# simon3dv/SLR-SFS

Measured on AMD Instinct MI355X. Metric: synthesised frames/sec at 768x1280 N=60, higher is better.
Workload: dtype f32 (convs: fp32 in/out/accumulate, operands 2 x f16 splits = 22 bits; all-fp32: fps_fp32_convs); 1 GPU; C3 baseline pipeline, 768x1280, N=60, random weights; parallelism=1 GPU, no collective, collective_bytes_received_per_rank_per_clip=0

## Files before the change

include/slr_splat.h:

```cpp
#ifndef SLR_SPLAT_H
#define SLR_SPLAT_H

#include <stddef.h>

#ifdef __cplusplus
extern "C" {
#endif

#define SLR_ABI_VERSION 28

#define SLR_E_BADARG   (-1)
#define SLR_E_WORKSPACE (-2)

#define SLR_MODE_SUMMATION 0
#define SLR_MODE_AVERAGE   1
#define SLR_MODE_LINEAR    2
#define SLR_MODE_SOFTMAX   3

#define SLR_NORM_ZERO_TO_ONE 0
#define SLR_NORM_CLAMP_EPS   1

int         slr_abi_version(void);
const char *slr_last_error(void);

void slr_splat_time_next(void *ev_start, void *ev_stop);


int slr_euler_integrate(const float *motion, int H, int W, int nsteps, float sign,
                        float *disp, float *visible, void *stream);

int slr_euler_integrate_all(const float *motion, int H, int W, int nmax, float sign,
                            float *disp_all, float *vis_all, void *stream);
// ... 114 lines not shown
                      int N, int C, int H, int W,
                      void *ws, size_t ws_bytes, int prebinned, void *stream);


int slr_bn_relu_mask(const float *x, const float *scale, const float *shift, const float *mask,
                     int mask_channels, float *y, int N, int C, int H, int W, void *stream);

int slr_pconv_epilogue(const float *raw0, const float *bias, const float *mask_box, float mask_scale,
                       const float *residual, const float *next_scale, const float *next_shift,
                       float *out, float *um_out, float winsize, int N, int C, int H, int W, void *stream);

int slr_conv_saturation_count(unsigned long long *count, int reset, void *stream);
int slr_conv_saturation_record(unsigned *host_slot, void *stream);


#define SLR_CONV_IN_B8  1
#define SLR_CONV_OUT_B8 2
#define SLR_CONV_RES_B8 4
#define SLR_CONV_F32    8
#define SLR_CONV_WINO   16
#define SLR_CONV_SKIP_B8 32
#define SLR_CONV_POOL_OUT 64
#define SLR_CONV_UP_OUT 128

size_t slr_conv3x3_weight_bytes(int Cout, int Cin);
int slr_conv3x3_split_weights(const float *w , void *wsplit, int Cout, int Cin,
                              float wscale, void *stream);
int slr_conv3x3_f32_weights(const float *w , void *wfrag , int Cout, int Cin,
                            void *stream);
size_t slr_conv3x3_wino_weight_bytes(int Cout, int Cin);
int slr_conv3x3_wino_weights(const float *w , void *wfrag , int Cout, int Cin,
                             void *stream);

int slr_conv3x3_forward(const float *in, const void *wsplit, const float *bias, const float *residual, float *out,
                        int N, int Cin, int Cout, int H, int W, float wscale, float xscale,
                        const float *pre_scale, const float *pre_shift, int layout, void *stream);

int slr_pconv3x3_forward(const float *x, const float *pre_scale, const float *pre_shift, const float *mask,
                         const void *wsplit, float wscale, float xscale, const float *bias, const float *residual,
                         const float *next_scale, const float *next_shift, float *out, float *um_out,
                         int N, int Cin, int Cout, int H, int W, int layout, void *stream);

size_t slr_conv_pool_ws_bytes(int N, int Cout, int H, int W);
size_t slr_conv_up_ws_bytes(int N, int Cout, int H, int W);
int slr_conv3x3_forward_skip(const float *in, const void *wsplit, const float *bias, float *out,
                             int N, int Cin, int Cout, int H, int W, float wscale, float xscale,
// ... 280 lines not shown
```

slr-sfs_amd/_lib.py:

```python
import ctypes
import os
import threading

import torch

_HERE = os.path.dirname(os.path.abspath(__file__))
LIB_PATH = os.environ.get("SLR_SFS_AMD_LIB") or os.path.join(_HERE, "lib", "libslrsplat.so")
ABI_VERSION = 28
WS_PREBINNED, WS_CLEAN = 1, 2
BLEND_DETERMINISTIC = 1

_vp, _fp, _i, _f, _sz = ctypes.c_void_p, ctypes.c_void_p, ctypes.c_int, ctypes.c_float, ctypes.c_size_t
SIGNATURES = {
    "slr_abi_version": (_i, []),
    "slr_last_error": (ctypes.c_char_p, []),
    "slr_splat_time_next": (None, [_vp, _vp]),
    "slr_euler_integrate": (_i, [_fp, _i, _i, _i, _f, _fp, _fp, _vp]),
    "slr_euler_integrate_all": (_i, [_fp, _i, _i, _i, _f, _fp, _fp, _vp]),
    "slr_euler_backward": (_i, [_fp, _i, _i, _i, _f, _fp, _fp, _vp]),
    "slr_euler_integrate_batch": (_i, [_fp, _vp, _i, _i, _i, _f, _fp, _fp, _vp]),
    "slr_euler_backward_batch": (_i, [_fp, _vp, _i, _i, _i, _f, _fp, _fp, _vp]),
    "slr_euler_pair_forward": (_i, [_fp, _vp, _vp, _i, _i, _i, _fp, _fp, _fp, _fp, _vp]),
    "slr_euler_pair_workspace_bytes": (_sz, [_i, _i, _i]),
    "slr_euler_pair_backward": (_i, [_fp, _vp, _vp, _i, _i, _i, _fp, _fp, _fp, _vp, _sz, _vp]),
    "slr_splat_workspace_bytes": (_sz, [_i, _i, _i]),
    "slr_splat_workspace_init": (_i, [_vp, _sz, _i, _i, _i, _vp]),
    "slr_splat_bin": (_i, [_fp, _i, _i, _i, _vp, _sz, _vp]),
    "slr_splat_bin_pair": (_i, [_fp, _fp, _i, _i, _i, _vp, _vp, _sz, _vp]),
    "slr_splat_set_scan_max_tiles": (_i, [_i]),
    "slr_splat_set_front_end": (_i, [_i]),
    "slr_splat_set_scan_shape": (None, [_i, _i, _i, _i]),
# ... 3 lines not shown
    "slr_synth_group": (_i, [_fp, _fp, _fp, _i, _fp, _fp, _f, _fp, _fp, _i, _i, _i, _f, _vp, _vp, _sz, _vp]),
    "slr_clip_plan_bytes": (_sz, [_i, _i, _i]),
    "slr_clip_plan_totals": (_i, [_i, _i, _i, ctypes.POINTER(ctypes.c_size_t), ctypes.POINTER(ctypes.c_int)]),
    "slr_clip_plan_build": (_i, [_fp, _vp, _fp, _vp, _i, _i, _i, _vp, _sz, _vp]),
    "slr_pack_planes4": (_i, [_fp, _fp, _i, _i, _i, _i, _vp]),
    "slr_synth_group_clip_batch": (_i, [_fp, _fp, _fp, _i, _vp, _vp, _vp, _vp, _vp, _i, _i, _i, _f, _vp, _sz, _i, _vp, _i, _vp, _vp]),
    "slr_synth_two_groups_clip_batch": (_i, [_fp, _fp, _fp, _i, _fp, _fp, _i, _vp, _vp, _vp, _vp, _vp, _i, _i, _i, _f, _vp, _sz, _i, _vp, _i, _vp, _vp]),
    "slr_synth_group_clip": (_i, [_fp, _fp, _fp, _i, _fp, _fp, _f, _fp, _fp, _i, _i, _i, _f, _vp, _sz, _i, _i, _i, _vp]),
    "slr_global_max": (_i, [_fp, _sz, _fp, _fp, _vp]),
    "slr_softsplat_backward": (_i, [_fp, _fp, _fp, _fp, _fp, _i, _i, _i, _i, _vp]),
    "slr_softsplat_backward_ws_bytes": (_sz, [_i, _i, _i, _i]),
    "slr_softsplat_backward_ws": (_i, [_fp, _fp, _fp, _fp, _fp, _i, _i, _i, _i, _vp, _sz, _vp]),
    "slr_splat_blend_ws_bytes": (_sz, [_i, _i, _i, _i]),
    "slr_splat_blend_forward": (_i, [_fp] * 9 + [_f, _f, _f, _fp, _fp, _i, _i, _i, _i, _vp, _sz, _i, _vp, _sz, _vp]),
    "slr_splat_blend_forward_ex": (_i, [_fp] * 9 + [_f, _f, _f, _fp, _fp, _i, _i, _i, _i, _vp, _sz, _i, _i, _vp, _sz, _vp]),
    "slr_splat_fallback_count_offset": (_sz, [_i, _i, _i]),
    "slr_splat_blend_backward": (_i, [_fp] * 9 + [_f, _f, _f] + [_fp] * 9 + [_i, _i, _i, _i, _vp, _sz, _vp]),
    "slr_maxsplat_forward": (_i, [_fp, _fp, _fp, _f, _i, _i, _i, _i, _vp, _sz, _i, _vp]),
    "slr_max_warp_norm": (_i, [_fp, _fp, _fp, _fp, _i, _i, _i, _i, _vp, _sz, _i, _vp]),
    "slr_bn_relu_mask": (_i, [_fp, _fp, _fp, _fp, _i, _fp, _i, _i, _i, _i, _vp]),
    "slr_pconv_epilogue": (_i, [_fp, _fp, _fp, _f, _fp, _fp, _fp, _fp, _fp, _f, _i, _i, _i, _i, _vp]),
    "slr_conv_saturation_count": (_i, [ctypes.POINTER(ctypes.c_ulonglong), _i, _vp]),
    "slr_conv_saturation_record": (_i, [_vp, _vp]),
    "slr_conv3x3_weight_bytes": (_sz, [_i, _i]),
    "slr_conv3x3_split_weights": (_i, [_fp, _vp, _i, _i, _f, _vp]),
    "slr_conv3x3_f32_weights": (_i, [_fp, _vp, _i, _i, _vp]),
    "slr_conv3x3_wino_weight_bytes": (_sz, [_i, _i]),
    "slr_conv3x3_wino_weights": (_i, [_fp, _vp, _i, _i, _vp]),
    "slr_conv3x3_forward": (_i, [_fp, _vp, _fp, _fp, _fp, _i, _i, _i, _i, _i, _f, _f, _fp, _fp, _i, _vp]),
    "slr_pconv3x3_forward": (_i, [_fp, _fp, _fp, _fp, _vp, _f, _f, _fp, _fp, _fp, _fp, _fp, _fp, _i, _i, _i, _i, _i, _i, _vp]),
    "slr_conv_pool_ws_bytes": (_sz, [_i, _i, _i, _i]),
    "slr_conv_up_ws_bytes": (_sz, [_i, _i, _i, _i]),
    "slr_conv3x3_forward_skip": (_i, [_fp, _vp, _fp, _fp, _i, _i, _i, _i, _i, _f, _f, _fp, _fp, _fp, _vp, _fp, _i, _f, _vp, _sz, _i, _vp]),
    "slr_pconv3x3_forward_skip": (_i, [_fp, _fp, _fp, _fp, _vp, _f, _f, _fp, _fp, _fp, _i, _i, _i, _i, _i, _fp, _vp, _i, _f, _vp, _sz, _i, _vp]),
    "slr_conv3x3_forward_skipout": (_i, [_fp, _vp, _fp, _fp, _fp, _i, _i, _i, _i, _i, _f, _f, _fp, _fp, _fp, _fp, _fp, _i, _vp]),
    "slr_pconv3x3_forward_skipout": (_i, [_fp, _fp, _fp, _fp, _vp, _f, _f, _fp, _fp, _fp, _fp, _fp, _fp, _i, _i, _i, _i, _i, _fp, _fp, _i, _vp]),
    "slr_conv_tail_weight_bytes": (_sz, [_i]),
    "slr_conv_tail_weight_source": (_i, [_i, _i, _vp, _vp, _vp, _vp]),
    "slr_conv_tail_weights": (_i, [_fp, _fp, _vp, _i, _f, _f, _vp]),
    "slr_pconv3x3_forward_tail": (_i, [_fp, _fp, _vp, _f, _f, _fp, _fp, _fp, _fp, _vp, _fp, _fp, _i, _i, _i, _i, _i, _vp]),
    "slr_narrow_gather": (_i, [_fp] * 9 + [_i, _i, _i, _i, _f, _f, _f, _vp]),
    "slr_conv1x1_weight_bytes": (_sz, [_i, _i]),
    "slr_conv1x1_split_weights": (_i, [_fp, _vp, _i, _i, _f, _vp]),
    "slr_conv1x1_f32_weights": (_i, [_fp, _vp, _i, _i, _vp]),
    "slr_conv1x1_forward": (_i, [_fp, _vp, _fp, _fp, _i, _i, _i, _i, _i, _f, _f, _i, _vp]),
    "slr_avgpool3x3s2": (_i, [_fp, _fp, _i, _i, _i, _i, _i, _vp]),
# ... 189 lines not shown
```

slr-sfs_amd/csrc/conv.hip:

```cpp
#include "slr_common.hpp"

#include <string.h>

#include <atomic>
#include <mutex>
#include <type_traits>

namespace slr {

typedef _Float16 h8 __attribute__((ext_vector_type(8)));
typedef float f16v __attribute__((ext_vector_type(16)));

constexpr int CV_W = 32, CV_H = 8;
constexpr int CV_HW = CV_W + 2, CV_HH = CV_H + 2;
constexpr int CV_NPX = CV_HW * CV_HH;
constexpr int CV_THREADS = 256;
constexpr float CV_XSCALE = 64.0f;
constexpr int CV_MAXCIN = 1024;

enum { PRE_NONE = 0, PRE_BN = 1, PRE_BN_MASK = 2, PRE_BN_NONZERO = 3 };

struct ConvArgs {
    const float *in;
    const h8 *w;
    float *out;
    int N, Cin, Cout, H, W, tiles_x, nchunk;
    float unscale;
    float xscale;
    int pre;
    const float *pre_scale, *pre_shift;
    const float *mask;
    const float *bias;
    int partial;
    float mask_scale, winsize;
    const float *residual, *next_scale, *next_shift;
    float *um_out;
    int out_b8;
    int res_b8;
// ... 2 lines not shown
    long long *trace;
#endif
    int wino_groups;
    const float *skip_in;
    const h8 *skip_w;
    const float *skip_bias;
    int skip_cin, skip_nchunk;
    float skip_unscale;
    float *pool_row, *pool_col;
    int tiles_y, resample;
    float *skip_out;
};

__host__ __device__ inline int conv_cout_tile(int Cout) { return Cout > 64 ? 128 : (Cout > 32 ? 64 : 32); }
__host__ __device__ inline int conv_cout_pad(int Cout) { const int t = conv_cout_tile(Cout); return (Cout + t - 1) / t * t; }
__host__ __device__ inline int conv_cin_pad(int Cin) { return (Cin + 15) / 16 * 16; }

}
#include "conv_few.hpp"
namespace slr {

constexpr int CV_FSTR = 352;
constexpr int CV_KSTR = 260;
template <int CPW, int WCO, bool PRE, bool INB8, bool F32 = false, bool SKIP = false, bool POOL = false, bool UPS = false, bool TAIL = false>
__global__ __launch_bounds__(CV_THREADS, 2) void conv3x3_split_kernel(ConvArgs a) {
    constexpr int WPX = 4 / WCO, PT = CV_H / WPX;
    static_assert(!TAIL || (CPW == 1 && WCO == 4 && !PRE && INB8 && !F32 && !SKIP && !POOL && !UPS), "the tail phase: one instantiation");
    static_assert(!(POOL || UPS) || (SKIP && WCO == 4 && !(POOL && UPS)), "the resampling epilogues: a wave holds all 8 rows of its channel tile");
    static_assert(!F32 || CPW == 1, "the fp32 rung runs one 32-channel tile per wave");
    static_assert(!SKIP || (CPW == 1 && INB8), "the skip phase: one tile per wave, channel-blocked main input");
    constexpr int XRAW = F32 ? 2 * 16 * CV_FSTR * 4 : 2 * 2 * 2 * CV_NPX * 16, XSKIP = !SKIP ? 0 : SLR_CONV_SKIP_FILL * (F32 ? 16 * CV_KSTR * 4 : 2 * 2 * 256 * 16);
    __shared__ __attribute__((aligned(16))) unsigned char xraw[XRAW > XSKIP ? XRAW : XSKIP];
    h8 (*xs)[2][2][CV_NPX] = reinterpret_cast<h8 (*)[2][2][CV_NPX]>(xraw);
    float (*xf)[16][CV_FSTR] = reinterpret_cast<float (*)[16][CV_FSTR]>(xraw);
    __shared__ float mpl[CV_NPX];
    __shared__ float mplB[2][CV_NPX - 256];
    __shared__ float4 pss4[2][CV_MAXCIN / 4];
    const int tid = threadIdx.x, lane = tid & 63;
    const int wave = __builtin_amdgcn_readfirstlane(tid >> 6);
    const int wc = wave % WCO, wp = wave / WCO;
    const int tx = blockIdx.x % a.tiles_x, ty = blockIdx.x / a.tiles_x;
    const int x0 = tx * CV_W, y0 = ty * CV_H;
    const int n = blockIdx.z;
    const int cot0 = (blockIdx.y * WCO + wc) * CPW;
    const int HW = a.H * a.W;
    const int nchunk = a.nchunk;
    const int cmax = a.Cin - 1;
    const float *inb = a.in + (size_t)n * a.Cin * HW;
    const int pre = a.pre;

    if (PRE) {
        float *pssw = reinterpret_cast<float *>(&pss4[0][0]);
        for (int i = tid; i < nchunk * 16; i += CV_THREADS) {
            pssw[i] = i < a.Cin ? a.pre_scale[i] * (F32 ? 1.0f : a.xscale) : 0.0f;
            pssw[CV_MAXCIN + i] = i < a.Cin ? a.pre_shift[i] * (F32 ? 1.0f : a.xscale) : 0.0f;
        }
    }

    const int gB = tid >= 84 ? 1 : 0;
    const int pB = 256 + tid - 84 * gB;
    const bool liveB = tid < 168;
    bool okA, okB;
    int offA, offB;
    {
        const int pr = tid / CV_HW, pc = tid - pr * CV_HW;
        const int gy = y0 - 1 + pr, gx = x0 - 1 + pc;
        okA = (gy >= 0) & (gy < a.H) & (gx >= 0) & (gx < a.W);
        offA = okA ? gy * a.W + gx : 0;
    }
    {
        const int pr = pB / CV_HW, pc = pB - pr * CV_HW;
        const int gy = y0 - 1 + pr, gx = x0 - 1 + pc;
        okB = liveB & (gy >= 0) & (gy < a.H) & (gx >= 0) & (gx < a.W);
        offB = okB ? gy * a.W + gx : 0;
    }
    const float unit = (PRE || F32) ? 1.0f : a.xscale;
    const float mvA = (a.mask && okA) ? a.mask[(size_t)n * HW + offA] : 0.0f;
    const float mvB = (a.mask && okB) ? a.mask[(size_t)n * HW + offB] : 0.0f;
    if (a.mask) {
        mpl[tid] = mvA;
        if (tid < CV_NPX - 256) mpl[256 + tid] = mvB;
    }
    const float mA = okA ? (pre == PRE_BN_MASK ? mvA : unit) : 0.0f;
    const float mB = okB ? (pre == PRE_BN_MASK ? mvB : unit) : 0.0f;
    float cnt[3] = {0.0f, 0.0f, 0.0f};
    const bool nonzero_mask = pre == PRE_BN_NONZERO;
    const int c8max = (a.Cin >> 3) - 1;
    auto load_round = [&](auto R, int c, float (&st)[8]) {
        if (INB8) {
            const int grp = min(c * 2 + (R.value < 2 ? R.value : gB), c8max);
            const float4 *q = reinterpret_cast<const float4 *>(inb) + ((size_t)grp * HW + (unsigned)(R.value < 2 ? offA : offB)) * 2;
            const float4 u = q[0], v = q[1];
            st[0] = u.x; st[1] = u.y; st[2] = u.z; st[3] = u.w;
            st[4] = v.x; st[5] = v.y; st[6] = v.z; st[7] = v.w;
            return;
        }
#pragma unroll
        for (int j = 0; j < 8; ++j) {
            if (R.value < 2) {
                const float *pl = inb + (size_t)min(c * 16 + R.value * 8 + j, cmax) * HW;
                st[j] = pl[(unsigned)offA];
            } else {
                st[j] = inb[(unsigned)(min(c * 16 + gB * 8 + j, cmax) * HW + offB)];
            }
        }
    };
    struct Stage { int cb; float mk0, fresh, cnt; h8 hi, lo; float f[F32 ? 8 : 1]; };
    unsigned long long sat = 0ull;
    const float *pss = reinterpret_cast<const float *>(&pss4[0][0]);
    auto stage_begin = [&](auto R, int c, Stage &g) {
        g.cb = c * 16 + (R.value < 2 ? R.value * 8 : gB * 8);
        g.mk0 = R.value < 2 ? mA : mB;
        g.cnt = 0.0f;
    };
    auto stage_value = [&](int j, Stage &g, const float (&st)[8], const float *psc = nullptr, const float *psh = nullptr) {
        const float x = st[j];
        float v;
        if (PRE) {
            const float mk = (nonzero_mask & (x == 0.0f)) ? 0.0f : g.mk0;
            v = fmaxf(x * (psc ? psc[j] : pss[g.cb + j]) - (psh ? psh[j] : pss[CV_MAXCIN + g.cb + j]), 0.0f) * mk;
            g.cnt += (g.cb + j <= cmax) ? mk : 0.0f;
        } else if (F32) {
            v = g.mk0 != 0.0f ? x : 0.0f;
        } else {
            v = x * g.mk0;
        }
        if (F32) { g.f[j] = v; return; }
        v = __builtin_amdgcn_fmed3f(v, -65472.0f, 65472.0f);
        sat |= __ballot(fabsf(v) >= 65472.0f);
        const _Float16 h = (_Float16)v;
        g.hi[j] = h;
        g.lo[j] = (_Float16)(v - (float)h);
    };
    auto stage_finish = [&](auto R, int buf, const Stage &g) {
        cnt[R.value] += g.cnt * g.fresh;
        const int dst = R.value == 0 ? tid : (R.value == 1 ? CV_NPX + tid : gB * CV_NPX + pB);
        if (F32) {
            const int ch0 = R.value < 2 ? R.value * 8 : gB * 8, px = R.value < 2 ? tid : pB;
            if (R.value < 2 || liveB) {
#pragma unroll
                for (int j = 0; j < 8; ++j) xf[buf][ch0 + j][px] = g.f[j];
            }
            return;
        }
        if (R.value < 2 || liveB) {
            (&xs[buf][0][0][0])[dst] = g.hi;
            (&xs[buf][1][0][0])[dst] = g.lo;
        }
    };
    auto store_round = [&](auto R, int buf, int c, const float (&st)[8]) {
        Stage g;
        stage_begin(R, c, g);
        g.fresh = 1.0f;
#pragma unroll
        for (int j = 0; j < 8; ++j) stage_value(j, g, st);
        stage_finish(R, buf, g);
    };
    using R0 = std::integral_constant<int, 0>;
    using R1 = std::integral_constant<int, 1>;
    using R2 = std::integral_constant<int, 2>;

    f16v acc[CPW][PT];
#pragma unroll
    for (int c = 0; c < CPW; ++c)
#pragma unroll
        for (int p = 0; p < PT; ++p)
#pragma unroll
            for (int r = 0; r < 16; ++r) acc[c][p][r] = 0.0f;

    __syncthreads();
    {
        float s0[8], s1[8], s2[8];
        load_round(R0{}, 0, s0);
        load_round(R1{}, 0, s1);
        load_round(R2{}, 0, s2);
        store_round(R0{}, 0, 0, s0);
        store_round(R1{}, 0, 0, s1);
        store_round(R2{}, 0, 0, s2);
    }
    __syncthreads();
    constexpr bool DEEP = SLR_CONV_DEEP_STAGE && WCO < 4 && !F32;
    float stx[DEEP ? 3 : 1][8];
    float (&st)[8] = stx[0];
    if (DEEP) load_round(R0{}, min(1, nchunk - 1), stx[0]);

    const int bcol = lane & 31, bgrp = lane >> 5;
    const size_t wtile = (size_t)nchunk * 9 * 2 * 64;
    const h8 *wbase = a.w + (size_t)cot0 * wtile;
    h8 a_cur[CPW][2], a_nxt[CPW][2];
    auto load_a = [&](h8 (&dst)[CPW][2], int g ) {
#pragma unroll
        for (int ct = 0; ct < CPW; ++ct) {
            const h8 *q = wbase + ct * wtile + (size_t)g * 128;
            if (F32) { dst[ct][0] = q[2u * (unsigned)lane]; dst[ct][1] = q[2u * (unsigned)lane + 1u]; continue; }
            dst[ct][0] = q[(unsigned)lane];
            dst[ct][1] = q[(unsigned)lane + 64u];
        }
    };
    load_a(a_cur, 0);
    const int glast = nchunk * 9 - 1;
    h8 a_nx2[DEEP ? CPW : 1][2];
    if (DEEP) { load_a(a_nxt, min(1, glast)); }
    constexpr int PB = PT > 4 ? 4 : PT, NB = PT / PB;
    constexpr int PSA = 2;
    for (int c = 0; c < nchunk; ++c) {
        const int buf = c & 1;
        h8 bx[2][PB];
        constexpr bool PSAHEAD = PRE && !F32;
        float psc[PSAHEAD ? 8 : 1], psh[PSAHEAD ? 8 : 1];
        const int cn = min(c + 1, nchunk - 1);
        const h8 *xh = &xs[buf][0][bgrp][0], *xl = &xs[buf][1][bgrp][0];
#pragma unroll
        for (int tap = 0; tap < 9; ++tap) {
            const int kh = tap / 3, kw = tap - kh * 3;
            asm volatile("" ::: "memory");
            if (DEEP) load_a(a_nx2, min(c * 9 + tap + 2, glast));
            else load_a(a_nxt, min(c * 9 + tap + 1, glast));
            if (DEEP) {
                if (tap == 0) load_round(R1{}, cn, stx[DEEP ? 1 : 0]);
                if (tap == 3) load_round(R2{}, cn, stx[DEEP ? 2 : 0]);
                if (tap == 6) load_round(R0{}, min(c + 2, nchunk - 1), stx[0]);
            } else {
                if (tap == 0) load_round(R0{}, cn, st);
                if (tap == 3) load_round(R1{}, cn, st);
                if (tap == 6) load_round(R2{}, cn, st);
            }
            __builtin_amdgcn_sched_barrier(0);
            const bool stage_tap = tap == 2 || tap == 5 || tap == 8;
            Stage sg;
            sg.fresh = c + 1 < nchunk ? 1.0f : 0.0f;
            if (stage_tap) {
                if (tap == 2) stage_begin(R0{}, cn, sg);
                if (tap == 5) stage_begin(R1{}, cn, sg);
                if (tap == 8) stage_begin(R2{}, cn, sg);
            }
            constexpr int NM = 3 * CPW * PT, NMB = 3 * CPW * PB;
            if constexpr (F32) {
                typedef float f8v __attribute__((ext_vector_type(8)));
                union AW { h8 h[2]; f8v f; } aw;
                aw.h[0] = a_cur[0][0]; aw.h[1] = a_cur[0][1];
                constexpr int NMF = 8 * PT;
#pragma unroll
                for (int kp = 0; kp < 8; ++kp) {
                    float bv[PT];
#pragma unroll
                    for (int k = 0; k < PT; ++k) bv[k] = xf[buf][2 * kp + bgrp][(wp * PT + k + kh) * CV_HW + kw + bcol];
#pragma unroll
                    for (int k = 0; k < PT; ++k) {
                        acc[0][k] = __builtin_amdgcn_mfma_f32_32x32x2f32(aw.f[kp], bv[k], acc[0][k], 0, 0, 0);
                        if (stage_tap) {
                            const int i = kp * PT + k;
                            const int j0 = i * 8 / NMF, j1 = (i + 1) * 8 / NMF;
                            if (j1 > j0) {
#pragma unroll
                                for (int j = j0; j < j1; ++j) stage_value(j, sg, stx[DEEP ? tap / 3 : 0]);
                                __builtin_amdgcn_sched_barrier(0);
                            }
                        }
                    }
                }
            } else {
                const int pcb = cn * 16 + (tap / 3 < 2 ? tap / 3 * 8 : gB * 8);
                auto ps_load = [&](int j) {
                    if constexpr (PSAHEAD) { psc[j] = pss[pcb + j]; psh[j] = pss[CV_MAXCIN + pcb + j]; }
                };
                auto frag = [&](int t, int b, int k) { return (wp * PT + b * PB + k + t / 3) * CV_HW + t % 3 + bcol; };
#pragma unroll
                for (int hb = 0; hb < NB; ++hb) {
                    const int q = (tap * NB + hb) & 1;
                    h8 (&bh)[PB] = bx[q], (&bl)[PB] = bx[q ^ 1];
                    if (tap == 0 && hb == 0) {
#pragma unroll
                        for (int k = 0; k < PB; ++k) {
                            bh[k] = xh[frag(0, 0, k)];
                            bl[k] = xl[frag(0, 0, k)];
                        }
                    }
                    const bool more = tap < 8 || hb + 1 < NB;
                    const int ntap = hb + 1 < NB ? tap : tap + 1, nhb = hb + 1 < NB ? hb + 1 : 0;
#pragma unroll
                    for (int ib = 0; ib < NMB; ++ib) {
                        const int part = ib / (CPW * PB), k = (ib / CPW) % PB, ct = ib % CPW;
                        const int pt = hb * PB + k, i = hb * NMB + ib;
                        const h8 av = part == 0 ? a_cur[ct][1] : a_cur[ct][0];
                        const h8 bv = part == 1 ? bl[k] : bh[k];
                        acc[ct][pt] = __builtin_amdgcn_mfma_f32_32x32x16_f16(av, bv, acc[ct][pt], 0, 0, 0);
                        if (more && ct == CPW - 1) {
                            if (part == 1) bl[k] = xh[frag(ntap, nhb, k)];
                            if (part == 2) bh[k] = xl[frag(ntap, nhb, k)];
                        }
                        if (tap % 3 == 1 && i == NM - PB - 1) {
#pragma unroll
                            for (int j = 0; j < PSA; ++j) ps_load(j);
                        }
                        if (stage_tap) {
                            const int j0 = i * 8 / NM, j1 = (i + 1) * 8 / NM;
#pragma unroll
                            for (int j = j0; j < j1; ++j) {
                                if (j + PSA < 8) ps_load(j + PSA);
                                if constexpr (PSAHEAD) stage_value(j, sg, stx[DEEP ? tap / 3 : 0], psc, psh);
                                else stage_value(j, sg, stx[DEEP ? tap / 3 : 0]);
                            }
                        }
                        __builtin_amdgcn_sched_barrier(0);
                    }
                }
            }
            if (stage_tap) {
                if (tap == 2) stage_finish(R0{}, buf ^ 1, sg);
                if (tap == 5) stage_finish(R1{}, buf ^ 1, sg);
                if (tap == 8) stage_finish(R2{}, buf ^ 1, sg);
            }
#pragma unroll
            for (int ct = 0; ct < CPW; ++ct) {
                a_cur[ct][0] = a_nxt[ct][0]; a_cur[ct][1] = a_nxt[ct][1];
                if (DEEP) { a_nxt[ct][0] = a_nx2[ct][0]; a_nxt[ct][1] = a_nx2[ct][1]; }
            }
        }
        __syncthreads();
    }

    if (pre == PRE_BN_NONZERO) {
        mpl[tid] = cnt[0] + cnt[1];
        if (liveB) mplB[gB][pB - 256] = cnt[2];
        __syncthreads();
        if (tid < CV_NPX - 256) mpl[256 + tid] = mplB[0][tid] + mplB[1][tid];
    }
    __syncthreads();

    if constexpr (SKIP) {
        constexpr int SK = SLR_CONV_SKIP_FILL;
        static_assert(SK * (F32 ? 16 * CV_KSTR * 4 : 2 * 2 * 256 * 16) <= (int)sizeof(xraw), "skip fills live in the staging buffers");
        h8 (*xk)[2][2][256] = reinterpret_cast<h8 (*)[2][2][256]>(xraw);
        float (*xkf)[16][CV_KSTR] = reinterpret_cast<float (*)[16][CV_KSTR]>(xraw);
        const int ns = a.skip_nchunk, sc8max = (a.skip_cin >> 3) - 1;
        const int spr = tid >> 5, spc = tid & 31;
        const bool sok = (y0 + spr < a.H) & (x0 + spc < a.W);
        const float smk = sok ? a.xscale : 0.0f;
        const float4 *sq = reinterpret_cast<const float4 *>(a.skip_in + (size_t)n * a.skip_cin * HW) + (size_t)(sok ? (y0 + spr) * a.W + x0 + spc : 0) * 2;
        float4 sv[SK][4];
        auto sload = [&](int s0) {
#pragma unroll
            for (int k = 0; k < SK; ++k)
#pragma unroll
                for (int g = 0; g < 2; ++g) {
                    const float4 *q = sq + (size_t)min(min(s0 + k, ns - 1) * 2 + g, sc8max) * HW * 2;
                    sv[k][2 * g] = q[0];
                    sv[k][2 * g + 1] = q[1];
                }
// ... 1131 lines not shown
    a.skip_in = sk->in; a.skip_w = (const h8 *)sk->w; a.skip_bias = sk->bias;
    a.skip_cin = sk->cin; a.skip_nchunk = conv_cin_pad(sk->cin) / 16;
    a.skip_unscale = 1.0f / (xscale * sk->wscale);
    if (pool) {
        SLR_CHECK_ARG(!(up && (layout_in & SLR_CONV_POOL_OUT)), "SLR_CONV_POOL_OUT and SLR_CONV_UP_OUT are exclusive");
        SLR_CHECK_ARG(a.out_b8 && conv_cout_tile(a.Cout) == 128, "the resampling epilogues need a channel-blocked output and more than 64 output channels");
        SLR_CHECK_ARG(!up || (long long)a.N * a.Cout * a.H * a.W < (1LL << 38), "sizes");
        SLR_CHECK_ARG(sk->pool_ws && !((uintptr_t)sk->pool_ws & 15) && sk->pool_ws_bytes >= conv_pool_ws_bytes(a.N, a.Cout, a.H, a.W, up),
                      "pool_ws: slr_conv_pool_ws_bytes / slr_conv_up_ws_bytes, 16-byte aligned");
        a.tiles_y = (a.H + CV_H - 1) / CV_H;
        a.resample = up ? 2 : 1;
        a.pool_row = (float *)sk->pool_ws;
        a.pool_col = a.pool_row + (size_t)a.N * a.Cout * a.tiles_y * a.W * (up ? 2 : 1);
    }
    return 0;
}

template <int WCO, bool PRE, bool B8, bool F32, bool SKIP, bool POOL, bool UPS>
static constexpr bool conv_split_built() {
    return !(WCO == 4 && PRE && !B8) && (B8 || !SKIP) && (!(POOL || UPS) || (SKIP && WCO == 4 && !(POOL && UPS))) &&
           !(F32 && SKIP && WCO != 4);
}

static int conv_launch(ConvArgs &a, float wscale, float xscale, int layout, hipStream_t st, bool tail = false) {
    const bool in_b8 = (layout & SLR_CONV_IN_B8) != 0, f32 = (layout & SLR_CONV_F32) != 0, wino = (layout & SLR_CONV_WINO) != 0;
    const bool pre = a.pre != PRE_NONE;
    if (int e = check_xscale(xscale)) return e;
    SLR_CHECK_ARG(!f32 || (wscale == 1.0f && xscale == 1.0f), "the fp32 rung takes no operand scales (wscale = xscale = 1)");
    SLR_CHECK_ARG(!wino || (f32 && a.Cout > CF_MAXCO), "SLR_CONV_WINO goes with SLR_CONV_F32 and more than 4 output channels");
    SLR_CHECK_ARG(!wino || !pre || a.Cin <= WN_MAXCIN, "SLR_CONV_WINO with a prologue supports Cin <= 256");
    if (wino) {
        a.tiles_x = (a.W + WN_BW - 1) / WN_BW;
        a.nchunk = conv_cin_pad(a.Cin) / 16;
        a.xscale = 1.0f; a.unscale = 1.0f;
        const int blocks = a.tiles_x * ((a.H + WN_BH - 1) / WN_BH), ngrp = wino_cout_pad(a.Cout) / 64;
        const dim3 grid((blocks + WN_SLICE - 1) / WN_SLICE * WN_SLICE * ngrp, 1, a.N);
        a.wino_groups = ngrp;
#ifdef SLR_TRACE
        a.trace = g_trace;
#endif
        if (int e = dispatch([&](auto pre_, auto b8) {
                static LdsOptIn attr;
                if (int e = lds_opt_in((const void *)conv3x3_wino_kernel<pre_, b8>, (int)WN_LDS_BYTES, attr)) return e;
                hipLaunchKernelGGL((conv3x3_wino_kernel<pre_, b8>), grid, dim3(WN_THREADS), WN_LDS_BYTES, st, a);
                return 0;
            }, pre, in_b8)) return e;
// ... 5 lines not shown
        if (int e = dispatch_int<1, 2, 3, 4>(a.Cout, [&](auto nco) {
                return dispatch([&](auto pre_, auto b8, auto skp) {
                    if constexpr (b8 || !skp) hipLaunchKernelGGL((conv3x3_few_kernel<nco, pre_, b8, skp>), grid, dim3(CF_THREADS), 0, st, a);
                    else return conv_not_built();
                    return 0;
                }, pre, in_b8, a.skip_out != nullptr);
            })) return e;
        SLR_CHECK_LAUNCH();
        return 0;
    }
    a.tiles_x = (a.W + CV_W - 1) / CV_W;
    a.nchunk = conv_cin_pad(a.Cin) / 16;
    a.xscale = xscale;
    a.unscale = 1.0f / (xscale * wscale);
    if (int e = sat_counter(&a.sat)) return e;
    if (tail) {
        hipLaunchKernelGGL((conv3x3_split_kernel<1, 4, false, true, false, false, false, false, true>),
                           dim3(a.tiles_x * ((a.H + CV_H - 1) / CV_H), 1, a.N), dim3(CV_THREADS), 0, st, a);
        SLR_CHECK_LAUNCH();
        return 0;
    }
    int ct = conv_cout_tile(a.Cout);
    if (ct == 128 && pre && !in_b8) ct = 64;
    const dim3 grid(a.tiles_x * ((a.H + CV_H - 1) / CV_H), conv_cout_pad(a.Cout) / ct, a.N);
    if (int e = dispatch_int<4, 2, 1>(ct / 32, [&](auto wco) {
            return dispatch([&](auto pre_, auto b8, auto f32_, auto skip, auto pool, auto ups) {
                if constexpr (conv_split_built<wco, pre_, b8, f32_, skip, pool, ups>())
                    hipLaunchKernelGGL((conv3x3_split_kernel<1, wco, pre_, b8, f32_, skip, pool, ups>), grid, dim3(CV_THREADS), 0, st, a);
                else return conv_not_built();
                return 0;
            }, pre, in_b8, f32, a.skip_in != nullptr, a.resample == 1, a.resample == 2);
        })) return e;
    SLR_CHECK_LAUNCH();
    if (a.resample == 2) {
        const int items = 2 * a.tiles_y * 2 * a.W + 2 * a.tiles_x * 2 * a.H;
        hipLaunchKernelGGL(upsample_fix_kernel, dim3((items + 255) / 256, a.N * (a.Cout >> 3)), dim3(256), 0, st, a.out, (const float *)a.pool_row,
                           (const float *)a.pool_col, a.Cout >> 3, a.H, a.W, a.tiles_x, a.tiles_y);
        SLR_CHECK_LAUNCH();
    } else if (a.resample == 1) {
        const int OH = (a.H - 1) / 2 + 1, OW = (a.W - 1) / 2 + 1;
        const int items = (a.tiles_y - 1) * OW + (a.tiles_x - 1) * OH;
        if (items > 0) {
            hipLaunchKernelGGL(pool_fix_kernel, dim3((items + 255) / 256, a.N * (a.Cout >> 3)), dim3(256), 0, st, a.out, (const float *)a.pool_row,
                               (const float *)a.pool_col, a.Cout >> 3, a.H, a.W, a.tiles_x, a.tiles_y);
            SLR_CHECK_LAUNCH();
        }
    }
    return 0;
}

static int conv3x3_run(bool partial, const float *x, const float *pre_scale, const float *pre_shift, const float *mask,
                       const void *wsplit, float wscale, float xscale, const float *bias, const float *residual,
                       const float *next_scale, const float *next_shift, float *out, float *um_out,
                       int N, int Cin, int Cout, int H, int W, const SkipOp *sk, int layout, void *stream) {
    SLR_CHECK_ARG(x && wsplit && (bias || !partial) && out, "null pointer");
    if (int e = conv_check_layout(layout, x, out, Cin, Cout, residual, partial && !mask)) return e;
    SLR_CHECK_ARG(!pre_scale == !pre_shift, "pre_scale / pre_shift go together");
    SLR_CHECK_ARG(!pre_scale || Cin <= CV_MAXCIN, "prologue supports Cin <= 1024");
    SLR_CHECK_ARG(!partial || mask || pre_scale, "mask = NULL (derived from x != 0) needs the raw input, i.e. pre_scale / pre_shift");
    SLR_CHECK_ARG(!next_scale == !next_shift, "next_scale / next_shift go together");
    SLR_CHECK_ARG(!(residual && next_scale), "residual and next-BN fusion are exclusive");
    if (int e = conv_check_dims(N, Cin, Cout, H, W)) return e;
    ConvArgs a = {};
    a.in = x; a.w = (const h8 *)wsplit; a.bias = bias; a.out = out;
    a.N = N; a.Cin = Cin; a.Cout = Cout; a.H = H; a.W = W;
    a.pre = !pre_scale ? PRE_NONE : !partial ? PRE_BN : mask ? PRE_BN_MASK : PRE_BN_NONZERO;
    a.pre_scale = pre_scale; a.pre_shift = pre_shift; a.mask = mask;
    if (partial) {
        a.partial = 1;
        a.mask_scale = mask ? (float)Cin : 1.0f;
        a.winsize = (float)Cin * 9.0f;
    }
    a.residual = residual; a.next_scale = next_scale; a.next_shift = next_shift; a.um_out = um_out;
    a.out_b8 = (layout & SLR_CONV_OUT_B8) != 0;
    a.res_b8 = (layout & SLR_CONV_RES_B8) != 0;
    if (int e = conv_set_skip(a, sk, xscale, layout)) return e;
    return conv_launch(a, wscale, xscale, layout, (hipStream_t)stream);
}

// ... 117 lines not shown
```

slr-sfs_amd/nets.py:

```python
import collections
import ctypes
import math
import types

import threading

import torch
import torch.nn as nn
import torch.nn.functional as F

from . import _lib


IN_B8, OUT_B8, RES_B8, CONV_F32, CONV_WINO, SKIP_B8, POOL_OUT, UP_OUT = 1, 2, 4, 8, 16, 32, 64, 128


class _Route(threading.local):
    cpu_reference = False
    torch_convs = False
    act_scale = 64.0
    f32_kernels = False
    winograd = False
    fused_skips = True
    fused_pools = True
    narrow_tail = True


_S = _Route()


def _b8(x, channels):
    return x.is_cuda and channels % 8 == 0 and not _S.torch_convs


class torch_convolutions:

    def __enter__(self):
        self._prev, _S.torch_convs = _S.torch_convs, True
        return self

    def __exit__(self, *exc):
        _S.torch_convs = self._prev
        return False


FP32_WINOGRAD = False


# ... 32 lines not shown

class staged_skips:

    def __init__(self, pools_only=False):
        self.pools_only = pools_only

    def __enter__(self):
        self._prev = (_S.fused_skips, _S.fused_pools)
        _S.fused_skips = self.pools_only
        _S.fused_pools = False

    def __exit__(self, *exc):
        _S.fused_skips, _S.fused_pools = self._prev
        return False


class staged_narrow_end:

    def __enter__(self):
        self._prev, _S.narrow_tail = _S.narrow_tail, False

    def __exit__(self, *exc):
        _S.narrow_tail = self._prev
        return False


_BlockRoute = collections.namedtuple("_BlockRoute", "form b8 first skip second pool")


def _block_route(blk, x, b8_in, explicit_mask=True):
    cout = blk.conv_aa.weight.shape[0]
    b8 = _b8(x, cout)
    lin = IN_B8 if b8_in else 0
    rides = blk.conv_b is not None and b8_in and _S.fused_skips and x.is_cuda and not _S.torch_convs
    if rides and cout <= 4 and explicit_mask:
        return _BlockRoute("narrow", b8, lin, 0, 0, False)
    first = lin | (OUT_B8 if b8 else 0)
    if rides and b8 and cout > 4 and not (_S.f32_kernels and (_S.winograd or cout <= 64)):
        return _BlockRoute("fused", b8, first, 0, IN_B8 | OUT_B8, blk.pools if (cout > 64 and _S.fused_pools) else False)
    skip_b8 = b8 and cout > 4 if blk.conv_b is not None else b8_in
    second = (IN_B8 | OUT_B8 if b8 else 0) | (RES_B8 if skip_b8 and b8 else 0)
    return _BlockRoute("staged", b8, first, lin | (OUT_B8 if skip_b8 else 0), second, False)


def _pool_out(N, cout, H, W, like, pool):
    if not pool:
# ... 102 lines not shown
        self.cin, self.k = cin, k
        nn.init.normal_(self.weight, std=math.sqrt(1.0 / (cin * k * k)))

    def forward(self, x, pre_bn=None, residual=None, layout=0):
        return self.conv(x, self.bias, pre_bn, residual, layout)

    def _w4(self):
        w = self.weight

        def make():
            w4 = torch.zeros(w.shape[1], 4, device=w.device, dtype=torch.float32)
            w4[:, :w.shape[0]] = w.view(w.shape[0], w.shape[1]).t()
            return w4.contiguous()
        return _cached(self, "_w4c", make, w)

    def _conv3x3(self, name, x, args, layout=0, pre_bn=None, next_bn=None, partial=False, skipout=False, skip_conv=None,
                 skip_b8=False, pool=False):
        N, cin, H, W = x.shape
        cout = self.weight.shape[0]
        c = types.SimpleNamespace(dims=(N, cin, cout, H, W), um=None, skip=None)
        c.buf, c.wscale, c.xscale, arith = self._split_weights()
        c.psc, c.psh = pre_bn if pre_bn is not None else (None, None)
        c.nsc, c.nsh = next_bn if next_bn is not None else (None, None)
        layout |= arith
        if skip_conv is not None:
            c.sbuf, c.swscale, _, sarith = skip_conv._split_weights()
            assert arith == sarith and not (arith & CONV_WINO)
            c.out, c.ws, c.ws_bytes, pflag = _pool_out(N, cout, H, W, x, pool)
            layout |= pflag | (SKIP_B8 if skip_b8 else 0)
        else:
            c.out = torch.empty(N, cout, H, W, device=x.device, dtype=x.dtype)
        if skipout:
            c.skip = torch.empty(N, cout, H, W, device=x.device, dtype=x.dtype)
        if partial:
            c.um = torch.empty(N, 1, H, W, device=x.device, dtype=x.dtype)
        _lib.call(name, x.device, *args(c), layout)
        return c

    def forward_skipout(self, x, pre_bn, skip_conv, layout=0):
        assert self.k == 3 and skip_conv.k == 1 and _fused_ok(x)
        c = self._conv3x3("slr_conv3x3_forward_skipout", x, lambda c: (
            x, c.buf, self.bias, None, c.out, *c.dims, c.wscale, c.xscale, c.psc, c.psh, skip_conv._w4(), skip_conv.bias, c.skip),
            layout, pre_bn, skipout=True)
        return c.out, c.skip

    def forward_skip(self, x, pre_bn, skip_x, skip_conv, layout=0, skip_b8=False, pool=False):
        assert self.k == 3 and skip_conv.k == 1 and _fused_ok(x, skip_x)
# ... 713 lines not shown
```

Before: 189.5 frames/s.

## Add 12-row tall conv tiles for 64-channel split convs on large grids

Adds a taller 32x12 spatial tile variant of the split-f16 3x3 conv kernel for 64-channel output tiles. It is chosen automatically when the grid has enough tiles per CU. The change generalises the halo staging from three to four load rounds, re-spaces the staging taps, and adjusts the MFMA pixel batching. The goal is to cut halo overhead, meaning redundant input loads and weight-fragment reloads per output pixel. The cost is more LDS and register pressure and fewer blocks, which could hurt occupancy or tail balance.

```diff
diff --git a/include/slr_splat.h b/include/slr_splat.h
--- a/include/slr_splat.h
+++ b/include/slr_splat.h
@@ -7,7 +7,7 @@
 extern "C" {
 #endif
 
-#define SLR_ABI_VERSION 28
+#define SLR_ABI_VERSION 29
 
 #define SLR_E_BADARG   (-1)
 #define SLR_E_WORKSPACE (-2)
@@ -168,6 +168,10 @@
 #define SLR_CONV_SKIP_B8 32
 #define SLR_CONV_POOL_OUT 64
 #define SLR_CONV_UP_OUT 128
+#define SLR_CONV_ROWS8 256
+#define SLR_CONV_ROWS_TALL 512
+
+int slr_conv_tile_rows(int Cout, int H, int W, int N, int layout, int num_cu);
 
 size_t slr_conv3x3_weight_bytes(int Cout, int Cin);
 int slr_conv3x3_split_weights(const float *w , void *wsplit, int Cout, int Cin,
diff --git a/slr-sfs_amd/_lib.py b/slr-sfs_amd/_lib.py
--- a/slr-sfs_amd/_lib.py
+++ b/slr-sfs_amd/_lib.py
@@ -6,7 +6,7 @@
 
 _HERE = os.path.dirname(os.path.abspath(__file__))
 LIB_PATH = os.environ.get("SLR_SFS_AMD_LIB") or os.path.join(_HERE, "lib", "libslrsplat.so")
-ABI_VERSION = 28
+ABI_VERSION = 29
 WS_PREBINNED, WS_CLEAN = 1, 2
 BLEND_DETERMINISTIC = 1
 
@@ -56,6 +56,7 @@
     "slr_pconv_epilogue": (_i, [_fp, _fp, _fp, _f, _fp, _fp, _fp, _fp, _fp, _f, _i, _i, _i, _i, _vp]),
     "slr_conv_saturation_count": (_i, [ctypes.POINTER(ctypes.c_ulonglong), _i, _vp]),
     "slr_conv_saturation_record": (_i, [_vp, _vp]),
+    "slr_conv_tile_rows": (_i, [_i] * 6),
     "slr_conv3x3_weight_bytes": (_sz, [_i, _i]),
     "slr_conv3x3_split_weights": (_i, [_fp, _vp, _i, _i, _f, _vp]),
     "slr_conv3x3_f32_weights": (_i, [_fp, _vp, _i, _i, _vp]),
diff --git a/slr-sfs_amd/csrc/conv.hip b/slr-sfs_amd/csrc/conv.hip
--- a/slr-sfs_amd/csrc/conv.hip
+++ b/slr-sfs_amd/csrc/conv.hip
@@ -12,8 +12,8 @@
 typedef float f16v __attribute__((ext_vector_type(16)));
 
 constexpr int CV_W = 32, CV_H = 8;
-constexpr int CV_HW = CV_W + 2, CV_HH = CV_H + 2;
-constexpr int CV_NPX = CV_HW * CV_HH;
+constexpr int CV_HW = CV_W + 2;
+constexpr int CV_H_TALL = 12;
 constexpr int CV_THREADS = 256;
 constexpr float CV_XSCALE = 64.0f;
 constexpr int CV_MAXCIN = 1024;
@@ -62,25 +62,32 @@
 
 constexpr int CV_FSTR = 352;
 constexpr int CV_KSTR = 260;
-template <int CPW, int WCO, bool PRE, bool INB8, bool F32 = false, bool SKIP = false, bool POOL = false, bool UPS = false, bool TAIL = false>
+template <int CPW, int WCO, bool PRE, bool INB8, bool F32 = false, bool SKIP = false, bool POOL = false, bool UPS = false, bool TAIL = false,
+          int TH = CV_H>
 __global__ __launch_bounds__(CV_THREADS, 2) void conv3x3_split_kernel(ConvArgs a) {
-    constexpr int WPX = 4 / WCO, PT = CV_H / WPX;
+    constexpr int WPX = 4 / WCO, PT = TH / WPX;
+    constexpr bool TALL = TH != CV_H;
+    constexpr int NPX = CV_HW * (TH + 2), REM = NPX - 256;
+    constexpr bool COMB = 2 * REM <= 256;
+    constexpr int NR = COMB ? 3 : 4;
+    static_assert(REM > 0 && REM <= 256, "the halo block: more than one and at most two rounds of pixels");
+    static_assert(!TALL || (CPW == 1 && WCO == 2 && !F32 && !SKIP && !POOL && !UPS && !TAIL), "the tall block: 64-channel rows of the split rung");
     static_assert(!TAIL || (CPW == 1 && WCO == 4 && !PRE && INB8 && !F32 && !SKIP && !POOL && !UPS), "the tail phase: one instantiation");
     static_assert(!(POOL || UPS) || (SKIP && WCO == 4 && !(POOL && UPS)), "the resampling epilogues: a wave holds all 8 rows of its channel tile");
     static_assert(!F32 || CPW == 1, "the fp32 rung runs one 32-channel tile per wave");
     static_assert(!SKIP || (CPW == 1 && INB8), "the skip phase: one tile per wave, channel-blocked main input");
-    constexpr int XRAW = F32 ? 2 * 16 * CV_FSTR * 4 : 2 * 2 * 2 * CV_NPX * 16, XSKIP = !SKIP ? 0 : SLR_CONV_SKIP_FILL * (F32 ? 16 * CV_KSTR * 4 : 2 * 2 * 256 * 16);
+    constexpr int XRAW = F32 ? 2 * 16 * CV_FSTR * 4 : 2 * 2 * 2 * NPX * 16, XSKIP = !SKIP ? 0 : SLR_CONV_SKIP_FILL * (F32 ? 16 * CV_KSTR * 4 : 2 * 2 * 256 * 16);
     __shared__ __attribute__((aligned(16))) unsigned char xraw[XRAW > XSKIP ? XRAW : XSKIP];
-    h8 (*xs)[2][2][CV_NPX] = reinterpret_cast<h8 (*)[2][2][CV_NPX]>(xraw);
+    h8 (*xs)[2][2][NPX] = reinterpret_cast<h8 (*)[2][2][NPX]>(xraw);
     float (*xf)[16][CV_FSTR] = reinterpret_cast<float (*)[16][CV_FSTR]>(xraw);
-    __shared__ float mpl[CV_NPX];
-    __shared__ float mplB[2][CV_NPX - 256];
+    __shared__ float mpl[NPX];
+    __shared__ float mplB[2][COMB ? REM : 1];
     __shared__ float4 pss4[2][CV_MAXCIN / 4];
     const int tid = threadIdx.x, lane = tid & 63;
     const int wave = __builtin_amdgcn_readfirstlane(tid >> 6);
     const int wc = wave % WCO, wp = wave / WCO;
     const int tx = blockIdx.x % a.tiles_x, ty = blockIdx.x / a.tiles_x;
-    const int x0 = tx * CV_W, y0 = ty * CV_H;
+    const int x0 = tx * CV_W, y0 = ty * TH;
     const int n = blockIdx.z;
     const int cot0 = (blockIdx.y * WCO + wc) * CPW;
     const int HW = a.H * a.W;
@@ -97,9 +104,9 @@
         }
     }
 
-    const int gB = tid >= 84 ? 1 : 0;
-    const int pB = 256 + tid - 84 * gB;
-    const bool liveB = tid < 168;
+    const int gB = COMB && tid >= REM ? 1 : 0;
+    const int pB = 256 + tid - REM * gB;
+    const bool liveB = tid < (COMB ? 2 * REM : REM);
     bool okA, okB;
     int offA, offB;
     {
@@ -119,16 +126,16 @@
     const float mvB = (a.mask && okB) ? a.mask[(size_t)n * HW + offB] : 0.0f;
     if (a.mask) {
         mpl[tid] = mvA;
-        if (tid < CV_NPX - 256) mpl[256 + tid] = mvB;
+        if (tid < REM) mpl[256 + tid] = mvB;
     }
     const float mA = okA ? (pre == PRE_BN_MASK ? mvA : unit) : 0.0f;
     const float mB = okB ? (pre == PRE_BN_MASK ? mvB : unit) : 0.0f;
-    float cnt[3] = {0.0f, 0.0f, 0.0f};
+    float cnt[NR] = {};
     const bool nonzero_mask = pre == PRE_BN_NONZERO;
     const int c8max = (a.Cin >> 3) - 1;
     auto load_round = [&](auto R, int c, float (&st)[8]) {
         if (INB8) {
-            const int grp = min(c * 2 + (R.value < 2 ? R.value : gB), c8max);
+            const int grp = min(c * 2 + (R.value < 2 ? R.value : (COMB ? gB : R.value - 2)), c8max);
             const float4 *q = reinterpret_cast<const float4 *>(inb) + ((size_t)grp * HW + (unsigned)(R.value < 2 ? offA : offB)) * 2;
             const float4 u = q[0], v = q[1];
             st[0] = u.x; st[1] = u.y; st[2] = u.z; st[3] = u.w;
@@ -137,9 +144,9 @@
         }
 #pragma unroll
         for (int j = 0; j < 8; ++j) {
-            if (R.value < 2) {
-                const float *pl = inb + (size_t)min(c * 16 + R.value * 8 + j, cmax) * HW;
-                st[j] = pl[(unsigned)offA];
+            if (R.value < 2 || !COMB) {
+                const float *pl = inb + (size_t)min(c * 16 + (R.value & 1) * 8 + j, cmax) * HW;
+                st[j] = pl[(unsigned)(R.value < 2 ? offA : offB)];
             } else {
                 st[j] = inb[(unsigned)(min(c * 16 + gB * 8 + j, cmax) * HW + offB)];
             }
@@ -149,7 +156,7 @@
     unsigned long long sat = 0ull;
     const float *pss = reinterpret_cast<const float *>(&pss4[0][0]);
     auto stage_begin = [&](auto R, int c, Stage &g) {
-        g.cb = c * 16 + (R.value < 2 ? R.value * 8 : gB * 8);
+        g.cb = c * 16 + (R.value < 2 ? R.value * 8 : (COMB ? gB * 8 : (R.value - 2) * 8));
         g.mk0 = R.value < 2 ? mA : mB;
         g.cnt = 0.0f;
     };
@@ -174,7 +181,7 @@
     };
     auto stage_finish = [&](auto R, int buf, const Stage &g) {
         cnt[R.value] += g.cnt * g.fresh;
-        const int dst = R.value == 0 ? tid : (R.value == 1 ? CV_NPX + tid : gB * CV_NPX + pB);
+        const int dst = R.value == 0 ? tid : (R.value == 1 ? NPX + tid : (COMB ? gB : R.value - 2) * NPX + pB);
         if (F32) {
             const int ch0 = R.value < 2 ? R.value * 8 : gB * 8, px = R.value < 2 ? tid : pB;
             if (R.value < 2 || liveB) {
@@ -199,6 +206,7 @@
     using R0 = std::integral_constant<int, 0>;
     using R1 = std::integral_constant<int, 1>;
     using R2 = std::integral_constant<int, 2>;
+    using R3 = std::integral_constant<int, 3>;
 
     f16v acc[CPW][PT];
 #pragma unroll
@@ -210,17 +218,19 @@
 
     __syncthreads();
     {
-        float s0[8], s1[8], s2[8];
+        float s0[8], s1[8], s2[8], s3[TALL ? 8 : 1];
         load_round(R0{}, 0, s0);
         load_round(R1{}, 0, s1);
         load_round(R2{}, 0, s2);
+        if constexpr (TALL) load_round(R3{}, 0, s3);
         store_round(R0{}, 0, 0, s0);
         store_round(R1{}, 0, 0, s1);
         store_round(R2{}, 0, 0, s2);
+        if constexpr (TALL) store_round(R3{}, 0, 0, s3);
     }
     __syncthreads();
-    constexpr bool DEEP = SLR_CONV_DEEP_STAGE && WCO < 4 && !F32;
-    float stx[DEEP ? 3 : 1][8];
+    constexpr bool DEEP = SLR_CONV_DEEP_STAGE && WCO < 4 && !F32 && !TALL;
+    float stx[DEEP ? 3 : (TALL ? 2 : 1)][8];
     float (&st)[8] = stx[0];
     if (DEEP) load_round(R0{}, min(1, nchunk - 1), stx[0]);
 
@@ -241,7 +251,7 @@
     const int glast = nchunk * 9 - 1;
     h8 a_nx2[DEEP ? CPW : 1][2];
     if (DEEP) { load_a(a_nxt, min(1, glast)); }
-    constexpr int PB = PT > 4 ? 4 : PT, NB = PT / PB;
+    constexpr int PB = PT > 4 ? PT / 2 : PT, NB = PT / PB;
     constexpr int PSA = 2;
     for (int c = 0; c < nchunk; ++c) {
         const int buf = c & 1;
@@ -256,7 +266,12 @@
             asm volatile("" ::: "memory");
             if (DEEP) load_a(a_nx2, min(c * 9 + tap + 2, glast));
             else load_a(a_nxt, min(c * 9 + tap + 1, glast));
-            if (DEEP) {
+            if constexpr (TALL) {
+                if (tap == 0) load_round(R0{}, cn, stx[0]);
+                if (tap == 1) load_round(R1{}, cn, stx[TALL ? 1 : 0]);
+                if (tap == 3) load_round(R2{}, cn, stx[0]);
+                if (tap == 5) load_round(R3{}, cn, stx[TALL ? 1 : 0]);
+            } else if (DEEP) {
                 if (tap == 0) load_round(R1{}, cn, stx[DEEP ? 1 : 0]);
                 if (tap == 3) load_round(R2{}, cn, stx[DEEP ? 2 : 0]);
                 if (tap == 6) load_round(R0{}, min(c + 2, nchunk - 1), stx[0]);
@@ -266,13 +281,22 @@
                 if (tap == 6) load_round(R2{}, cn, st);
             }
             __builtin_amdgcn_sched_barrier(0);
-            const bool stage_tap = tap == 2 || tap == 5 || tap == 8;
+            const bool stage_tap = TALL ? tap >= 2 && tap % 2 == 0 : tap == 2 || tap == 5 || tap == 8;
+            const int sround = TALL ? (tap + 1) / 2 - 1 : tap / 3;
+#define CV_STAGE_SET (DEEP ? tap / 3 : (TALL ? sround & 1 : 0))
             Stage sg;
             sg.fresh = c + 1 < nchunk ? 1.0f : 0.0f;
             if (stage_tap) {
-                if (tap == 2) stage_begin(R0{}, cn, sg);
-                if (tap == 5) stage_begin(R1{}, cn, sg);
-                if (tap == 8) stage_begin(R2{}, cn, sg);
+                if constexpr (TALL) {
+                    if (tap == 2) stage_begin(R0{}, cn, sg);
+                    if (tap == 4) stage_begin(R1{}, cn, sg);
+                    if (tap == 6) stage_begin(R2{}, cn, sg);
+                    if (tap == 8) stage_begin(R3{}, cn, sg);
+                } else {
+                    if (tap == 2) stage_begin(R0{}, cn, sg);
+                    if (tap == 5) stage_begin(R1{}, cn, sg);
+                    if (tap == 8) stage_begin(R2{}, cn, sg);
+                }
             }
             constexpr int NM = 3 * CPW * PT, NMB = 3 * CPW * PB;
             if constexpr (F32) {
@@ -293,14 +317,14 @@
                             const int j0 = i * 8 / NMF, j1 = (i + 1) * 8 / NMF;
                             if (j1 > j0) {
 #pragma unroll
-                                for (int j = j0; j < j1; ++j) stage_value(j, sg, stx[DEEP ? tap / 3 : 0]);
+                                for (int j = j0; j < j1; ++j) stage_value(j, sg, stx[CV_STAGE_SET]);
                                 __builtin_amdgcn_sched_barrier(0);
                             }
                         }
                     }
                 }
             } else {
-                const int pcb = cn * 16 + (tap / 3 < 2 ? tap / 3 * 8 : gB * 8);
+                const int pcb = cn * 16 + (TALL ? (sround < 2 ? (sround > 0 ? sround : 0) : sround - 2) * 8 : (tap / 3 < 2 ? tap / 3 * 8 : gB * 8));
                 auto ps_load = [&](int j) {
                     if constexpr (PSAHEAD) { psc[j] = pss[pcb + j]; psh[j] = pss[CV_MAXCIN + pcb + j]; }
                 };
@@ -329,7 +353,7 @@
                             if (part == 1) bl[k] = xh[frag(ntap, nhb, k)];
                             if (part == 2) bh[k] = xl[frag(ntap, nhb, k)];
                         }
-                        if (tap % 3 == 1 && i == NM - PB - 1) {
+                        if ((TALL ? tap % 2 == 1 : tap % 3 == 1) && i == NM - PB - 1) {
 #pragma unroll
                             for (int j = 0; j < PSA; ++j) ps_load(j);
                         }
@@ -338,8 +362,8 @@
 #pragma unroll
                             for (int j = j0; j < j1; ++j) {
                                 if (j + PSA < 8) ps_load(j + PSA);
-                                if constexpr (PSAHEAD) stage_value(j, sg, stx[DEEP ? tap / 3 : 0], psc, psh);
-                                else stage_value(j, sg, stx[DEEP ? tap / 3 : 0]);
+                                if constexpr (PSAHEAD) stage_value(j, sg, stx[CV_STAGE_SET], psc, psh);
+                                else stage_value(j, sg, stx[CV_STAGE_SET]);
                             }
                         }
                         __builtin_amdgcn_sched_barrier(0);
@@ -347,9 +371,16 @@
                 }
             }
             if (stage_tap) {
-                if (tap == 2) stage_finish(R0{}, buf ^ 1, sg);
-                if (tap == 5) stage_finish(R1{}, buf ^ 1, sg);
-                if (tap == 8) stage_finish(R2{}, buf ^ 1, sg);
+                if constexpr (TALL) {
+                    if (tap == 2) stage_finish(R0{}, buf ^ 1, sg);
+                    if (tap == 4) stage_finish(R1{}, buf ^ 1, sg);
+                    if (tap == 6) stage_finish(R2{}, buf ^ 1, sg);
+                    if (tap == 8) stage_finish(R3{}, buf ^ 1, sg);
+                } else {
+                    if (tap == 2) stage_finish(R0{}, buf ^ 1, sg);
+                    if (tap == 5) stage_finish(R1{}, buf ^ 1, sg);
+                    if (tap == 8) stage_finish(R2{}, buf ^ 1, sg);
+                }
             }
 #pragma unroll
             for (int ct = 0; ct < CPW; ++ct) {
@@ -359,12 +390,17 @@
         }
         __syncthreads();
     }
+#undef CV_STAGE_SET
 
     if (pre == PRE_BN_NONZERO) {
         mpl[tid] = cnt[0] + cnt[1];
-        if (liveB) mplB[gB][pB - 256] = cnt[2];
-        __syncthreads();
-        if (tid < CV_NPX - 256) mpl[256 + tid] = mplB[0][tid] + mplB[1][tid];
+        if constexpr (COMB) {
+            if (liveB) mplB[gB][pB - 256] = cnt[2];
+            __syncthreads();
+            if (tid < REM) mpl[256 + tid] = mplB[0][tid] + mplB[1][tid];
+        } else {
+            if (liveB) mpl[256 + tid] = cnt[2] + cnt[NR - 1];
+        }
     }
     __syncthreads();
 
@@ -1542,6 +1578,30 @@
            !(F32 && SKIP && WCO != 4);
 }
 
+constexpr int CV_TALL_MIN_ROUNDS = 4;
+static int conv_tile_rows(int Cout, int H, int W, int N, int layout, int num_cu) {
+    if ((layout & (SLR_CONV_F32 | SLR_CONV_WINO | SLR_CONV_SKIP_B8 | SLR_CONV_ROWS8)) || conv_cout_tile(Cout) != 64) return CV_H;
+    if (layout & SLR_CONV_ROWS_TALL) return CV_H_TALL;
+    const long long tiles = (long long)((W + CV_W - 1) / CV_W) * ((H + CV_H_TALL - 1) / CV_H_TALL) * N;
+    return tiles >= (long long)CV_TALL_MIN_ROUNDS * 2 * num_cu ? CV_H_TALL : CV_H;
+}
+
+SLR_EXPORT int slr_conv_tile_rows(int Cout, int H, int W, int N, int layout, int num_cu) {
+    if (Cout <= 0 || H <= 0 || W <= 0 || N <= 0 || num_cu <= 0) return 0;
+    return conv_tile_rows(Cout, H, W, N, layout, num_cu);
+}
+
+static int conv_num_cu(int *cu) {
+    static std::atomic<int> known[64] = {};
+    int dev = 0;
+    SLR_CHECK_HIP(hipGetDevice(&dev));
+    const bool tracked = dev >= 0 && dev < 64;
+    if (tracked && (*cu = known[dev].load(std::memory_order_relaxed)) > 0) return 0;
+    SLR_CHECK_HIP(hipDeviceGetAttribute(cu, hipDeviceAttributeMultiprocessorCount, dev));
+    if (tracked) known[dev].store(*cu, std::memory_order_relaxed);
+    return 0;
+}
+
 static int conv_launch(ConvArgs &a, float wscale, float xscale, int layout, hipStream_t st, bool tail = false) {
     const bool in_b8 = (layout & SLR_CONV_IN_B8) != 0, f32 = (layout & SLR_CONV_F32) != 0, wino = (layout & SLR_CONV_WINO) != 0;
     const bool pre = a.pre != PRE_NONE;
@@ -1593,6 +1653,20 @@
     }
     int ct = conv_cout_tile(a.Cout);
     if (ct == 128 && pre && !in_b8) ct = 64;
+    if (ct == 64 && !f32 && !a.skip_in) {
+        int cu = 0;
+        if (!(layout & (SLR_CONV_ROWS8 | SLR_CONV_ROWS_TALL)))
+            if (int e = conv_num_cu(&cu)) return e;
+        if (conv_tile_rows(a.Cout, a.H, a.W, a.N, layout, cu) == CV_H_TALL) {
+            const dim3 grid(a.tiles_x * ((a.H + CV_H_TALL - 1) / CV_H_TALL), conv_cout_pad(a.Cout) / ct, a.N);
+            if (int e = dispatch([&](auto pre_, auto b8) {
+                    hipLaunchKernelGGL((conv3x3_split_kernel<1, 2, pre_, b8, false, false, false, false, false, CV_H_TALL>), grid, dim3(CV_THREADS), 0, st, a);
+                    return 0;
+                }, pre, in_b8)) return e;
+            SLR_CHECK_LAUNCH();
+            return 0;
+        }
+    }
     const dim3 grid(a.tiles_x * ((a.H + CV_H - 1) / CV_H), conv_cout_pad(a.Cout) / ct, a.N);
     if (int e = dispatch_int<4, 2, 1>(ct / 32, [&](auto wco) {
             return dispatch([&](auto pre_, auto b8, auto f32_, auto skip, auto pool, auto ups) {
@@ -1625,7 +1699,8 @@
                        const float *next_scale, const float *next_shift, float *out, float *um_out,
                        int N, int Cin, int Cout, int H, int W, const SkipOp *sk, int layout, void *stream) {
     SLR_CHECK_ARG(x && wsplit && (bias || !partial) && out, "null pointer");
-    if (int e = conv_check_layout(layout, x, out, Cin, Cout, residual, partial && !mask)) return e;
+    SLR_CHECK_ARG((layout & (SLR_CONV_ROWS8 | SLR_CONV_ROWS_TALL)) != (SLR_CONV_ROWS8 | SLR_CONV_ROWS_TALL), "SLR_CONV_ROWS8 and SLR_CONV_ROWS_TALL are exclusive");
+    if (int e = conv_check_layout(layout & ~(SLR_CONV_ROWS8 | SLR_CONV_ROWS_TALL), x, out, Cin, Cout, residual, partial && !mask)) return e;
     SLR_CHECK_ARG(!pre_scale == !pre_shift, "pre_scale / pre_shift go together");
     SLR_CHECK_ARG(!pre_scale || Cin <= CV_MAXCIN, "prologue supports Cin <= 1024");
     SLR_CHECK_ARG(!partial || mask || pre_scale, "mask = NULL (derived from x != 0) needs the raw input, i.e. pre_scale / pre_shift");
diff --git a/slr-sfs_amd/nets.py b/slr-sfs_amd/nets.py
--- a/slr-sfs_amd/nets.py
+++ b/slr-sfs_amd/nets.py
@@ -13,6 +13,7 @@
 
 
 IN_B8, OUT_B8, RES_B8, CONV_F32, CONV_WINO, SKIP_B8, POOL_OUT, UP_OUT = 1, 2, 4, 8, 16, 32, 64, 128
+ROWS8, ROWS_TALL = 256, 512
 
 
 class _Route(threading.local):
@@ -24,6 +25,7 @@
     fused_skips = True
     fused_pools = True
     narrow_tail = True
+    conv_rows = 0
 
 
 _S = _Route()
@@ -102,6 +104,19 @@
 
     def __exit__(self, *exc):
         _S.narrow_tail = self._prev
+        return False
+
+
+class eight_row_tiles:
+
+    def __init__(self, tall=False):
+        self.flag = ROWS_TALL if tall else ROWS8
+
+    def __enter__(self):
+        self._prev, _S.conv_rows = _S.conv_rows, self.flag
+
+    def __exit__(self, *exc):
+        _S.conv_rows = self._prev
         return False
 
 
@@ -250,7 +265,7 @@
         c.buf, c.wscale, c.xscale, arith = self._split_weights()
         c.psc, c.psh = pre_bn if pre_bn is not None else (None, None)
         c.nsc, c.nsh = next_bn if next_bn is not None else (None, None)
-        layout |= arith
+        layout |= arith | _S.conv_rows
         if skip_conv is not None:
             c.sbuf, c.swscale, _, sarith = skip_conv._split_weights()
             assert arith == sarith and not (arith & CONV_WINO)
```

Result: no change. 190.3 frames/s (median of 6 runs) (+0.5%).
